# zhxie0117/video-tokenizer

Hardware: AMD Instinct MI355X
Metric: clips/sec (16x128x128) tokenizer fwd+bwd (higher is better)
Workload: dtype bf16; 1 GPU; cfgs/larp_tokenizer.yaml base geometry as LARPTokenizer(bottleneck_type=vq): config B, 16x128x128 clips, 8 clips/GPU, 12+12 blocks, Nq=1024, d=24, K=8192, stochastic VQ (tau 0.03), loss = L1 + 0.1*loss_q; global_batch=8, parallelism=dp1

## Files before the change

### include/vt_hip.h

```cpp
#ifndef VT_HIP_H
#define VT_HIP_H
#include <stddef.h>
#include <stdint.h>
#ifdef __cplusplus
extern "C" {
#endif

typedef void* vtStream;

enum { VT_OK = 0, VT_ERR_INVALID = -1, VT_ERR_LAUNCH = -2, VT_ERR_UNSUPPORTED = -3 };

int vt_abi_version(void);
int vt_last_error(char* buf, size_t n);

typedef struct {
    int32_t grp;
    int64_t stride;
    int64_t off;
} vtRowMap;

enum {
    VT_EPI_BF16 = 0,
    VT_EPI_BF16_GELU = 1,
    VT_EPI_F32 = 2,
// ... 8 lines not shown
    int32_t M, N, K;
    int32_t epi;
    void* out; int64_t ldo;
    void* out2; int64_t ldo2;
    const float* bias;
    const float* residual; int64_t ldr;
    const float* rowmod; int32_t rowmod_period;
    const void* aux; int64_t ldaux;
    vtRowMap omap;
    int32_t round_bf16;
    float* colsum_partial;
    float out_scale;
    int32_t tile;
    void* splitk_ws; int64_t splitk_ws_bytes;
    int32_t splitk;
} vtGemmNT;
size_t vt_gemm_nt_splitk_workspace_bytes(void);

int vt_gemm_nt(const vtGemmNT* p_host, vtStream stream);

#define VT_TN_MAX_GROUP 16
typedef struct {
    const void* A; int64_t lda;
    const void* B; int64_t ldb;
    int32_t M, P, Q;
    float* out; int64_t ldo;
    int32_t p_lim, q_lim;
    const int32_t* row_perm;
    int32_t tile;
} vtGemmTN;
// ... 322 lines not shown
```

### video-tokenizer_amd/csrc/vt_attention.hip

```cpp
#include "vt_common.h"
#include <stdlib.h>

#include <type_traits>

#include "vt_attn_tile.h"

namespace {

struct AttnOps {
    const bf16_t *q, *k, *v;
    int64_t q_rs, k_rs, v_rs;
    int Lq, Lk;
};
struct AttnGrads {
    bf16_t *dq, *dk, *dv;
    int64_t dq_rs, dk_rs, dv_rs;
};
struct HeadPtrs {
    int blk;
    int Lq, Lk;
    int hq, hkv;
    int group;
    int64_t qrow, krow;
    int64_t q_rs, k_rs, v_rs, ors;
// ... 277 lines not shown
            sacc[r] = ds[0];
            sacc[r + 1] = ds[1];
        }
#pragma unroll
        for (int sp = 0; sp < 2; ++sp) {
            const bf16x8 dsf = pack8(sacc, sp);
#pragma unroll
            for (int dt = 0; dt < HD / 32; ++dt)
                dq[dt] = __builtin_amdgcn_mfma_f32_32x32x16_bf16(trfrag_a<HD>(kl, ad, kt * 32, sp, dt), dsf, dq[dt], 0, 0, 0);
        }
    }
}

template <int KS>
__device__ __forceinline__ float delta_own(const bf16x8 (&of)[KS], const bf16x8 (&dof)[KS]) {
    float d = 0.f;
#pragma unroll
    for (int s = 0; s < KS; ++s)
#pragma unroll
        for (int j = 0; j < 8; ++j) d += bf2f(of[s][j]) * bf2f(dof[s][j]);
    d += __shfl_xor(d, 32);
    return d;
}

template <int HD, bool CAUSAL, bool CROSS, bool OWN_DELTA, class Heads>
__device__ __forceinline__ void attn_bwd_dq_body(Heads&& heads, const bf16_t* __restrict__ o, const bf16_t* __restrict__ dO,
                                                 const float* __restrict__ lse2, std::conditional_t<OWN_DELTA, float, const float>* __restrict__ delta,
                                                 const AttnGrads grads, float scale, float scale_log2e, int q_begin) {
    extern __shared__ __attribute__((aligned(16))) char smem[];
    const int tid = threadIdx.x, lane = tid & 63;
    const int wave = __builtin_amdgcn_readfirstlane(tid >> 6);
    const int half = lane >> 5;
    const HeadPtrs hp = heads();
    const int Lq = hp.Lq, Lk = hp.Lk;
    const int q0 = q_begin + hp.blk * 128 + wave * 32;
// ... 280 lines not shown

template <int HD>
constexpr int kDqLds = 4 * AG<HD>::TILE;
template <int HD>
constexpr int kDkvLds = 2 * (2 * AG<HD>::TILE + 512);

template <int HD, bool CROSS = false>
static void launch_bwd(const AttnOps& ops, const void* o, const void* dO, const float* lse2, int B, int H, int q_begin, const AttnGrads& grads,
                       float* delta_ws, hipStream_t s) {
    if (q_begin > 0) {
        const int64_t n = (int64_t)B * q_begin * (H * HD / 8);
        hipLaunchKernelGGL(zero_q_rows_kernel, dim3((unsigned)((n + 255) / 256)), dim3(256), 0, s, grads.dq, ops.Lq, q_begin, (int64_t)3 * H * HD, H * HD);
    }
    const int nblk_q = (ops.Lq - q_begin + 127) / 128, nblk_k = (ops.Lk + 127) / 128;
    const int n_dq = nblk_q * B * H, n_dkv = nblk_k * B * H;
    hipLaunchKernelGGL((attn_delta_kernel<HD, CROSS>), dim3(n_dq), dim3(256), 0, s, ops, (const bf16_t*)o, (const bf16_t*)dO, delta_ws, H, nblk_q,
                       q_begin);
    hipLaunchKernelGGL((attn_bwd_kernel<HD, CROSS>), dim3(n_dkv + n_dq), dim3(256), kDqLds<HD> > kDkvLds<HD> ? kDqLds<HD> : kDkvLds<HD>, s, ops,
                       (const bf16_t*)dO, lse2, delta_ws, grads, H, nblk_q, nblk_k, n_dkv, kScale<HD>, kScaleLog2e<HD>, q_begin);
}
static void launch_causal_bwd(const AttnOps& ops, const void* o, const void* dO, const float* lse2, int B, int H, const AttnGrads& grads,
                              float* delta_ws, hipStream_t s) {
    const int nblk = (ops.Lq + 127) / 128;
    hipLaunchKernelGGL(attn_causal_bwd_dq_kernel, dim3(nblk * B * H), dim3(256), kDqLds<64>, s, ops, (const bf16_t*)o, (const bf16_t*)dO, lse2,
                       delta_ws, grads, H, nblk, kScale<64>, kScaleLog2e<64>);
    hipLaunchKernelGGL(attn_causal_bwd_dkv_kernel, dim3(nblk * B * H), dim3(256), kDkvLds<64>, s, ops, (const bf16_t*)dO, lse2, delta_ws, grads, H,
                       nblk, kScale<64>, kScaleLog2e<64>);
}

static bool attn_aligned(const void* a, const void* b = nullptr, const void* c = nullptr, const void* d = nullptr) {
    return ((((uintptr_t)a) | ((uintptr_t)b) | ((uintptr_t)c) | ((uintptr_t)d)) & 15) == 0;
}
// ... 8 lines not shown

extern "C" int vt_attention_fwd_rows(const void* qkv, int32_t B, int32_t L, int32_t H, int32_t hd, int32_t q_begin, void* o_compact, float* lse2,
                                     vtStream stream) {
    VT_CHECK_ARG(qkv && o_compact && lse2, "vt_attention_fwd: null pointer");
    VT_CHECK_ARG(attn_aligned(qkv, o_compact), "vt_attention_fwd: qkv and o must be 16-byte aligned");
    int rc = attn_check("vt_attention_fwd", B, L, H, hd, q_begin);
    if (rc) return rc;
    if (hd == 64) launch_fwd<64>(packed_ops(qkv, L), B, H, q_begin, o_compact, lse2, (hipStream_t)stream);
    else launch_fwd<32>(packed_ops(qkv, L), B, H, q_begin, o_compact, lse2, (hipStream_t)stream);
    VT_CHECK_LAUNCH("vt_attention_fwd");
    return VT_OK;
}

extern "C" int vt_attention_bwd_rows(const void* qkv, const void* o_compact, const void* dO_compact, const float* lse2, int32_t B, int32_t L,
                                     int32_t H, int32_t hd, int32_t q_begin, void* dqkv, float* delta_ws, vtStream stream) {
    VT_CHECK_ARG(qkv && o_compact && dO_compact && lse2 && dqkv && delta_ws, "vt_attention_bwd: null pointer");
    VT_CHECK_ARG(attn_aligned(qkv, o_compact, dO_compact, dqkv), "vt_attention_bwd: qkv, o, dO and dqkv must be 16-byte aligned");
    int rc = attn_check("vt_attention_bwd", B, L, H, hd, q_begin);
    if (rc) return rc;
    if (hd == 64) launch_bwd<64>(packed_ops(qkv, L), o_compact, dO_compact, lse2, B, H, q_begin, packed_grads(dqkv), delta_ws, (hipStream_t)stream);
    else launch_bwd<32>(packed_ops(qkv, L), o_compact, dO_compact, lse2, B, H, q_begin, packed_grads(dqkv), delta_ws, (hipStream_t)stream);
    VT_CHECK_LAUNCH("vt_attention_bwd");
    return VT_OK;
}

extern "C" int vt_attention_fwd(const void* qkv, int32_t B, int32_t L, int32_t H, int32_t hd, void* o, float* lse2, vtStream stream) {
    return vt_attention_fwd_rows(qkv, B, L, H, hd, 0, o, lse2, stream);
}

extern "C" int vt_attention_bwd(const void* qkv, const void* o, const void* dO, const float* lse2, int32_t B, int32_t L, int32_t H,
                                int32_t hd, void* dqkv, float* delta_ws, vtStream stream) {
// ... 140 lines not shown
```

### video-tokenizer_amd/csrc/vt_common.h

```cpp
#pragma once
#include <hip/hip_runtime.h>
#include <stdint.h>
#include <stdio.h>
#include <string.h>

#include "../../include/vt_hip.h"

typedef __bf16 bf16_t;
typedef __attribute__((ext_vector_type(8))) __bf16 bf16x8;
typedef __attribute__((ext_vector_type(4))) __bf16 bf16x4;
typedef __attribute__((ext_vector_type(2))) __bf16 bf16x2;
typedef __attribute__((ext_vector_type(4))) short s16x4;
typedef __attribute__((ext_vector_type(2))) float f32x2;
typedef __attribute__((ext_vector_type(4))) float f32x4;
typedef __attribute__((ext_vector_type(16))) float f32x16;

#define VT_LDS __attribute__((address_space(3)))
#define VT_GLB __attribute__((address_space(1)))

void vt_set_error(const char* fmt, ...);
#define VT_CHECK_ARG(cond, ...)                 \
    do {                                        \
        if (!(cond)) {                          \
            vt_set_error(__VA_ARGS__);          \
// ... 144 lines not shown
    const int q = nwg >> 3, r = nwg & 7, x = bid & 7;
    const int base = (x < r) ? x * (q + 1) : r * (q + 1) + (x - r) * q;
    return base + (bid >> 3);
}

static inline int vt_auto_col_block(int tiles_n, int in_flight) {
    if (tiles_n < 2 || in_flight < 4) return 0;
    int target = 1;
    while ((target + 1) * (target + 1) <= in_flight) ++target;
    if ((target + 1) * (target + 1) - in_flight < in_flight - target * target) ++target;
    int k = (tiles_n + target / 2) / target;
    if (k < 1) k = 1;
    const int w = (tiles_n + k - 1) / k;
    return w >= tiles_n ? 0 : w;
}
__host__ __device__ __forceinline__ void vt_tile_of(int sid, int tiles_m, int tiles_n, int col_block, int& tm, int& tn) {
    tm = sid / tiles_n, tn = sid - tm * tiles_n;
    if (col_block > 0) {
        const int per = tiles_m * col_block, b = sid / per, r = sid - b * per;
        const int left = tiles_n - b * col_block, w = left < col_block ? left : col_block;
        tm = r / w, tn = b * col_block + (r - tm * w);
    }
}

struct RowMap {
    int grp;
    int64_t stride, off;
    __host__ __device__ __forceinline__ int64_t operator()(int64_t r) const {
        return grp ? (r / grp) * stride + off + (r % grp) : r;
    }
// ... 18 lines not shown
```

### video-tokenizer_amd/csrc/vt_engine.hip

```cpp
#include <vector>

#include "vt_common.h"

extern "C" int vt_kl_forward(const float* z, int64_t ldz, int64_t M, int32_t d, int32_t batch, uint64_t seed, const uint32_t* seed_counter,
                             float* mean, float* sample, void* sample_pad_bf16, int64_t ldp, float* noise, float* loss_kl, void* workspace,
                             vtStream stream) __attribute__((weak));
extern "C" int vt_kl_backward(const float* g_sample, int64_t ldg, const float* g_mean, const float* gkl, const float* z, int64_t ldz,
                              const float* noise, int64_t M, int32_t d, int32_t batch, float* dz, void* dz_pad_bf16, int64_t ldp,
                              vtStream stream) __attribute__((weak));
extern "C" int vt_rope_rotate(void* qkv, int64_t ld, int64_t M, int32_t L, int32_t H, const float* cos_tab, const float* sin_tab,
                              int32_t conjugate, vtStream stream) __attribute__((weak));

static const bool g_no_splitk = [] { const char* e = getenv("VT_GEMM_SPLITK"); return e && strcmp(e, "0") == 0; }();

namespace {

__global__ void gather_f32_kernel(const float* __restrict__ src, const int32_t* __restrict__ perm, int n, float* __restrict__ dst) {
    const int i = blockIdx.x * blockDim.x + threadIdx.x;
    if (i < n) dst[i] = src[perm[i]];
}
__global__ void scatter_f32_kernel(const float* __restrict__ src, const int32_t* __restrict__ perm, int n, float* __restrict__ dst) {
    const int i = blockIdx.x * blockDim.x + threadIdx.x;
    if (i < n) dst[perm[i]] = src[i];
}
// ... 206 lines not shown
        t->vq_ws = a.take(vt_vq_workspace_bytes(t->Mq, c.K, c.d));
    }
    t->encoded_int = a.take(Mqp * D * 4);
    t->hN = a.take(Mvp * D * 2); t->meanH = a.take(Mvp * 4); t->rstdH = a.take(Mvp * 4);
    t->yrows = a.take(Mvp * Kp * 4);
    for (Side* sd : {&t->enc, &t->dec}) {
        const int nk = sd == &t->enc ? c.Nq : t->Nv, q_begin = t->L - nk;
        sd->last.rows = Rows{{nk, t->L, q_begin}, c.B * nk, (int)round_up(c.B * nk, 128), q_begin};
        sd->last.enabled = q_begin % 64 == 0 && q_begin > 0;
    }
    plan_block_scratch(t, a, {&t->enc, &t->dec}, (int)(Kp > (size_t)t->D4 ? Kp : t->D4));
    t->dY = a.take(Mvp * Kp * 2); t->dhN = a.take(Mvp * D * 2);
    t->dEncb = a.take(Mqp * D * 2); t->d_rz = a.take(Mqp * 64 * 4); t->dz_pad = a.take(Mqp * 64 * 2);
    t->dTok = a.take(Mvp * D * 2);
    t->tmp_vec = a.take((Kp > (size_t)t->D4 ? Kp : t->D4) * 4);
    t->wg_slabs = a.take((size_t)16 * D * 64 * 4);
    t->ws_bytes = a.off;
    *out = t;
    return VT_OK;
}

extern "C" int vt_tokenizer_create(const vtTokenizerConfig* cfg, vtTokenizer** out) { return create_tokenizer(cfg, false, out); }
extern "C" int vt_tokenizer_create_kl(const vtTokenizerConfig* cfg, vtTokenizer** out) { return create_tokenizer(cfg, true, out); }

extern "C" void vt_tokenizer_destroy(vtTokenizer* t) { delete t; }
extern "C" size_t vt_tokenizer_workspace_bytes(const vtTokenizer* t) { return t ? t->ws_bytes : 0; }
extern "C" int32_t vt_tokenizer_num_backward_stages(const vtTokenizer* t) { return t ? 3 + t->c.depth_enc + t->c.depth_dec : 0; }
static int set_split_k(BlockEngine* e, int32_t on, const char* fn) {
    VT_CHECK_ARG(e, "%s: null handle", fn);
    e->splitk_on = on != 0;
    return VT_OK;
// ... 230 lines not shown
                         WS(float, t->meanH), WS(float, t->rstdH), s));
    vtGemmNT g = nt(t, ws, WS(void, t->hN), D, WS(void, t->head_wb), D, t->Mv, t->Kp, D, VT_EPI_F32, WS(void, t->yrows), t->Kp);
    g.bias = WS(float, t->head_b_perm);
    TRY(vt_gemm_nt(&g, s));
    TRY(vt_unpatchify(WS(float, t->yrows), c.B, c.C, c.T, c.S, c.pt, c.p, pred, s));
    return VT_OK;
}

static vtGemmTN tn(const void* A, int64_t lda, const void* B, int64_t ldb, int M, int P, int Q, float* out, int64_t ldo) {
    vtGemmTN p;
    memset(&p, 0, sizeof(p));
    p.A = A; p.lda = lda; p.B = B; p.ldb = ldb; p.M = M; p.P = P; p.Q = Q; p.out = out; p.ldo = ldo; p.p_lim = P; p.q_lim = Q;
    return p;
}

static int skinny_wgrad(vtTokenizer* t, vtGemmTN w, void* ws, vtStream s) {
    int ns = 16;
    while (ns > 1 && (w.M % (64 * ns)) != 0) ns >>= 1;
    if (ns == 1) return vt_gemm_tn_grouped(&w, 1, s);
    const int rows = w.M / ns;
    const size_t slab = (size_t)w.p_lim * w.q_lim;
    vtGemmTN pr[16];
    float* part = WS(float, t->wg_slabs);
    for (int i = 0; i < ns; ++i) {
        pr[i] = w;
        pr[i].A = (const char*)w.A + (size_t)i * rows * w.lda * 2;
        pr[i].B = (const char*)w.B + (size_t)i * rows * w.ldb * 2;
        pr[i].M = rows;
        pr[i].out = part + i * slab;
        pr[i].ldo = w.q_lim;
    }
    TRY(vt_gemm_tn_grouped(pr, ns, s));
// ... 77 lines not shown
    void* dqkv = WS(void, g0.dqkv);
    if (kept) TRY(vt_cast_rows(dX, r.map, r.n, D, dXa, D, s));
    vtGemmNT g = nt(e, ws, dXa, D, WS(void, b.fc2_wt), D, r.n, D4, D, VT_EPI_BF16_MULAUX, du, D4);
    g.aux = WS(void, b.dgelu); g.ldaux = D4;
    g.colsum_partial = WS(float, g0.cs_part);
    TRY(vt_gemm_nt(&g, s));
    queue_slab_sum(e, WS(float, g0.cs_part), (r.n + 191) / 192, D4, gr.fc1_b);
    g = nt(e, ws, du, D4, WS(void, b.fc1_wt), D4, r.n, D, D4, VT_EPI_BF16, WS(void, e->dh), D);
    TRY(vt_gemm_nt(&g, s));
    int nsl = 0;
    TRY(vt_layernorm_bwd_partials(WS(void, e->dh), WS(float, b.x_mid), r.map, w.norm2_w, WS(float, b.mean2), WS(float, b.rstd2), dX, r.n, D, dX,
                                  kept ? nullptr : dXm, WS(float, g0.ln_part2), &nsl, s));
    queue_ln_reduce(e, WS(float, g0.ln_part2), nsl, D, gr.norm2_w, gr.norm2_b, gr.proj_b);
    if (kept) TRY(vt_cast_rows(dX, r.map, r.n, D, dXm, D, s));
    g = nt(e, ws, dXm, D, WS(void, b.proj_wt), D, r.n, D, D, VT_EPI_BF16, WS(void, e->dob), D);
    TRY(vt_gemm_nt(&g, s));
    TRY(attn_bwd(e, ws, WS(void, b.qkv), WS(void, b.o), WS(void, e->dob), WS(float, b.lse), r.q_begin, dqkv, s));
    if (rope_cos) TRY(vt_rope_rotate(dqkv, D3, M, e->L, e->H, rope_cos, rope_sin, 1, s));
    g = nt(e, ws, dqkv, D3, WS(void, b.qkv_wt), D3, M, D, D3, VT_EPI_BF16, WS(void, e->dh), D);
    TRY(vt_gemm_nt(&g, s));
    e->pending.push_back(tn(dXa, D, WS(void, b.g), D4, r.n_pad, D, D4, gr.fc2_w, D4));
    e->pending.push_back(tn(du, D4, WS(void, b.h2), D, r.n_pad, D4, D, gr.fc1_w, D));
    e->pending.push_back(tn(dXm, D, WS(void, b.o), D, r.n_pad, D, D, gr.proj_w, D));
    e->pending.push_back(tn(dqkv, D3, WS(void, b.h1), D, Mp, D3, D, gr.qkv_w, D));
    e->pending_blocks++;
    TRY(vt_layernorm_bwd_partials(WS(void, e->dh), x_in, id, w.norm1_w, WS(float, b.mean1), WS(float, b.rstd1), dX, M, D, dX, WS(void, g1.dx_out),
                                  WS(float, g0.ln_part1), &nsl, s));
    queue_ln_reduce(e, WS(float, g0.ln_part1), nsl, D, gr.norm1_w, gr.norm1_b, prev_bias_grad);
    e->set_idx = set_next;
    return VT_OK;
}

// ... 34 lines not shown
            t->pending_red.clear(); t->pending_blocks = 0; t->set_idx = 0; t->final_through = 0;
            t->sets_pending.clear();
            TRY(join_wgrad_stream(t, s));
            VT_CHECK_ARG(d_pred, "vt_tokenizer_backward: stage 0 needs d_pred");
            TRY(vt_patchify(d_pred, c.B, c.C, c.T, c.S, c.pt, c.p, WS(void, t->dY), s));
            vtGemmNT g = nt(t, ws, WS(void, t->dY), Kp, WS(void, t->head_wt), Kp, t->Mv, D, Kp, VT_EPI_BF16, WS(void, t->dhN), D);
            TRY(vt_gemm_nt(&g, s));
            vtGemmTN w = tn(WS(void, t->dY), Kp, WS(void, t->hN), D, t->Mvp, Kp, D, G->head_w, D);
            w.row_perm = WS(int32_t, t->perm);
            TRY(vt_gemm_tn_grouped(&w, 1, s));
            TRY(vt_colsum(WS(void, t->dY), 1, Kp, id, t->Mv, Kp, WS(float, t->tmp_vec), WS(void, t->cs_ws), s));
            hipLaunchKernelGGL(scatter_f32_kernel, dim3((Kp + 255) / 256), dim3(256), 0, hs, WS(float, t->tmp_vec), WS(int32_t, t->perm), Kp, G->head_b);
            TRY(vt_zero_rows(dX, WS(void, t->gs[0].dx_out), lmap, t->Mq, D, s));
            TRY(vt_layernorm_bwd(WS(void, t->dhN), WS(float, t->dec.x[c.depth_dec]), vmap, P->head_norm_w, WS(float, t->meanH), WS(float, t->rstdH),
                                 nullptr, t->Mv, D, dX, WS(void, t->gs[0].dx_out), G->head_norm_w, G->head_norm_b,
                                 nullptr, WS(void, t->ln_ws), s));
            TRY(vt_colsum(dX, 0, D, id, t->M, D, G->dec_blocks[c.depth_dec - 1].fc2_b, WS(void, t->cs_ws), s));
            t->final_through = 1;
        } else if (st <= c.depth_dec) {
            const int i = c.depth_dec - st;
            TRY(backward_block_stage(t, t->dec, i, P->dec_blocks, G->dec_blocks, true, false, st + 1, ws, s));
        } else if (st == c.depth_dec + 1) {
            if (G->dec_token_type) TRY(vt_colsum(dX, 0, D, vmap, t->Mv, D, G->dec_token_type, WS(void, t->cs_ws), s));
            TRY(vt_cast_rows(dX, lmap, t->Mq, D, WS(void, t->dEncb), D, s));
            TRY(vt_colsum(WS(void, t->dEncb), 1, D, id, t->Mq, D, G->out_b, WS(void, t->cs_ws), s));
            vtGemmNT g = nt(t, ws, WS(void, t->dEncb), D, WS(void, t->out_wt), D, t->Mq, 64, D, VT_EPI_F32, WS(void, t->d_rz), 64);
            TRY(vt_gemm_nt(&g, s));
            vtGemmTN w = tn(WS(void, t->dEncb), D, WS(void, t->vq_rzpad), 64, t->Mqp, D, 64, G->out_w, c.d);
            w.q_lim = c.d;
            TRY(skinny_wgrad(t, w, ws, s));
            const int pd = t->kl ? 2 * c.d : c.d;
            if (t->kl) {
// ... 12 lines not shown
            TRY(wait_set(t, t->set_idx, s));
            TRY(vt_zero_rows(dX, WS(void, t->gs[t->set_idx].dx_out), tmap, t->Mv, D, s));
            g = nt(t, ws, WS(void, t->dz_pad), 64, WS(void, t->in_wt), 64, t->Mq, D, 64, VT_EPI_F32, dX, D);
            g.out2 = WS(void, t->gs[t->set_idx].dx_out); g.ldo2 = D; g.omap = qmap;
            TRY(vt_gemm_nt(&g, s));
            TRY(vt_colsum(dX, 0, D, id, t->M, D, G->enc_blocks[c.depth_enc - 1].fc2_b, WS(void, t->cs_ws), s));
            t->final_through = st + 1;
        } else if (st <= c.depth_dec + 1 + c.depth_enc) {
            const int i = c.depth_enc - (st - c.depth_dec - 1);
            TRY(backward_block_stage(t, t->enc, i, P->enc_blocks, G->enc_blocks, true, i < t->wg_tail, st + 1, ws, s));
        } else {
            TRY(vt_batch_sum(dX, qmap, c.B, Nq, D, G->enc_query, s));
            TRY(vt_cast_rows(dX, tmap, t->Mv, D, WS(void, t->dTok), D, s));
            TRY(vt_colsum(WS(void, t->dTok), 1, D, id, t->Mv, D, G->pe_b, WS(void, t->cs_ws), s));
            vtGemmTN w = tn(WS(void, t->dTok), D, WS(void, t->patches), Kp, t->Mvp, D, Kp, G->pe_w, Kp);
            TRY(vt_gemm_tn_grouped(&w, 1, s));
            TRY(join_wgrad_stream(t, s));
            t->final_through = st + 1;
        }
    }
    if (final_through) *final_through = t->final_through;
    VT_CHECK_LAUNCH("vt_tokenizer_backward");
    return VT_OK;
}

extern "C" int vt_tokenizer_backward_until_flush(vtTokenizer* t, const vtTokenizerTensors* P, const float* d_pred, const float* gscal, void* ws,
                                                 const vtTokenizerTensors* G, int32_t stage_begin, int32_t* stage_next, int32_t* final_through,
                                                 vtStream s) {
    VT_CHECK_ARG(t && stage_next && final_through, "vt_tokenizer_backward_until_flush: null pointer");
    const int nstage = vt_tokenizer_num_backward_stages(t);
    VT_CHECK_ARG(stage_begin >= 0 && stage_begin < nstage, "vt_tokenizer_backward_until_flush: bad first stage");
// ... 96 lines not shown
```

### video-tokenizer_amd/csrc/vt_gemm.hip

```cpp
#include "vt_common.h"
#include "vt_gemm_epilogue.h"

namespace {

constexpr int BM = 128, BN = 128, BK = 64;
constexpr int TILE_B = BM * BK * 2;

struct NTArgs {
    vtGemmNT p;
    int tiles_m, tiles_n;
    int col_block;
    int split;
    float* part;
    unsigned* ctr;
};

__device__ __forceinline__ void st_part(float* p, const f32x4& v) {
    asm volatile("global_store_dwordx4 %0, %1, off sc1\n\ts_nop 1" ::"v"(p), "v"(v) : "memory");
}

__device__ __forceinline__ void stage_nt(const bf16_t* __restrict__ g, int64_t ld, int row0, int nrows, int k0,
                                         char* lds, int tid, int wave) {
#pragma unroll
    for (int i = 0; i < 4; ++i) {
// ... 465 lines not shown
    VT_CHECK_ARG(p.M > 0 && p.N > 0 && p.K > 0 && p.K % BK == 0, "vt_gemm_nt: K=%d must be a positive multiple of 64 (M=%d N=%d)", p.K, p.M, p.N);
    VT_CHECK_ARG(p.lda % 8 == 0 && p.ldb % 8 == 0 && p.lda >= p.K && p.ldb >= p.K, "vt_gemm_nt: lda/ldb must be >= K and multiples of 8");
    VT_CHECK_ARG(((uintptr_t)p.A & 15) == 0 && ((uintptr_t)p.B & 15) == 0, "vt_gemm_nt: A/B must be 16-byte aligned");
    VT_CHECK_ARG(p.ldo % 4 == 0, "vt_gemm_nt: ldo must be a multiple of 4");
    VT_CHECK_ARG(((uintptr_t)p.out & 15) == 0 && ((uintptr_t)p.bias & 15) == 0 && ((uintptr_t)p.out2 & 7) == 0 &&
                 ((uintptr_t)p.residual & 15) == 0 && ((uintptr_t)p.rowmod & 15) == 0 && ((uintptr_t)p.aux & 7) == 0,
                 "vt_gemm_nt: out/bias/residual/rowmod must be 16-byte aligned (out2/aux 8-byte)");
    VT_CHECK_ARG(!p.rowmod || p.N % 4 == 0, "vt_gemm_nt: rowmod needs N %% 4 == 0");
    if (p.epi == VT_EPI_BF16_GELU) VT_CHECK_ARG(p.out2 && p.ldo2 % 4 == 0, "vt_gemm_nt: GELU epilogue needs out2");
    if (p.epi == VT_EPI_BF16_GELU_GRAD) VT_CHECK_ARG(p.out2 && p.ldo2 % 4 == 0, "vt_gemm_nt: GELU_GRAD epilogue needs out2");
    if (p.epi == VT_EPI_BF16_DGELU) VT_CHECK_ARG(p.aux && p.ldaux % 4 == 0, "vt_gemm_nt: DGELU epilogue needs aux");
    if (p.epi == VT_EPI_BF16_MULAUX) VT_CHECK_ARG(p.aux && p.ldaux % 4 == 0, "vt_gemm_nt: MULAUX epilogue needs aux");
    VT_CHECK_ARG(p.out_scale == 0.f || p.epi == VT_EPI_F32, "vt_gemm_nt: out_scale only with VT_EPI_F32");
    VT_CHECK_ARG(!p.colsum_partial || ((p.epi == VT_EPI_BF16_DGELU || p.epi == VT_EPI_BF16_MULAUX) && p.N % 4 == 0),
                 "vt_gemm_nt: colsum_partial needs the DGELU or MULAUX epilogue and N %% 4 == 0 (it always runs on the 192-row tile kernel)");
    if (p.epi == VT_EPI_F32) {
        VT_CHECK_ARG(!p.residual || p.ldr % 4 == 0, "vt_gemm_nt: ldr must be a multiple of 4");
        VT_CHECK_ARG(!p.rowmod || p.rowmod_period > 0, "vt_gemm_nt: rowmod needs a period");
        VT_CHECK_ARG(!p.out2 || p.ldo2 % 4 == 0, "vt_gemm_nt: ldo2 must be a multiple of 4");
    } else {
        VT_CHECK_ARG(p.omap.grp == 0, "vt_gemm_nt: output row map only with VT_EPI_F32");
    }
    if (tile.kernel == NTTile::SKINNY || (tile.kernel == NTTile::AUTO && p.M <= 64 && !p.colsum_partial && p.N >= 64)) {
        VT_CHECK_ARG(p.M <= 64 && !p.colsum_partial, "vt_gemm_nt: tile 7 (skinny) needs M <= 64 and no colsum_partial (M=%d)", p.M);
        hipStream_t s = (hipStream_t)stream;
        TRY(dispatch_epi(p.epi, [&](auto epi) { launch_skinny<decltype(epi)::value>(p, s); return VT_OK; }));
        VT_CHECK_LAUNCH("vt_gemm_nt(skinny)");
        return VT_OK;
    }
    bool big = tile.kernel == NTTile::T192 || p.colsum_partial;
    if (tile.kernel == NTTile::AUTO && !big && p.N >= 192 && p.M >= 192) {
        const long t192 = (long)((p.M + 191) / 192) * ((p.N + 191) / 192), t128 = (long)((p.M + BM - 1) / BM) * ((p.N + BN - 1) / BN);
        const double c192 = (double)((t192 + 255) / 256);
        const long rem = t128 % 512;
        const double last = rem == 0 ? 0.0 : rem <= 256 ? 0.6 : 0.6 + 0.4 * (double)(rem - 256) / 256.0;
        const double c128 = 1.05 * ((double)(t128 / 512) + last);
        big = c192 <= c128;
    }
    if (big) {
        TRY(vt_gemm192_init());
        TRY(vt_gemm_nt192_launch(p, (hipStream_t)stream, tile.one_tile, tile.order));
        VT_CHECK_LAUNCH("vt_gemm_nt(192)");
        return VT_OK;
    }
    NTArgs a;
    a.p = p;
    a.tiles_m = (p.M + BM - 1) / BM;
    a.tiles_n = (p.N + BN - 1) / BN;
    a.split = 1; a.part = nullptr; a.ctr = nullptr;
    const int tiles = a.tiles_m * a.tiles_n;
    hipStream_t s = (hipStream_t)stream;
    const int n_cu = vt_gemm_num_cus();
    const int nt_all = p.K / BK;
// ... 78 lines not shown
```

### video-tokenizer_amd/csrc/vt_gemm192.hip

```cpp
#include <stdlib.h>

#include "vt_common.h"
#include "vt_gemm_epilogue.h"

namespace {

constexpr int TM = 192, TN_ = 192, TK = 64;
constexpr int OP_BYTES = TM * TK * 2;
constexpr int STAGE_BYTES = 2 * OP_BYTES;
constexpr int NSTAGE = 3;
constexpr int THREADS = 512;
constexpr int PA = 3, PB = 3, P = PA + PB;

__device__ __forceinline__ void wait_vmcnt6() { asm volatile("s_waitcnt vmcnt(6)" ::: "memory"); }
static_assert(P == 6 && PA * THREADS == TM * 8 && PB * THREADS == TN_ * 8, "wait_vmcnt6 counts one K-tile");
__device__ __forceinline__ void wait_vmcnt0() { asm volatile("s_waitcnt vmcnt(0)" ::: "memory"); }
__device__ __forceinline__ void raw_barrier() {
    asm volatile("" ::: "memory");
    __builtin_amdgcn_s_barrier();
    asm volatile("" ::: "memory");
}

struct NT192Args {
    vtGemmNT p;
// ... 67 lines not shown
        for (int g = 0; g < 3; ++g) {
            const int m = m0 + row, n = n0 + col0 + g * 64;
            if (m >= p.M || n >= p.N) continue;
            V* const o = (V*)((bf16_t*)p.out + (int64_t)m * p.ldo + n);
            auto o2 = [&] { return (V*)((bf16_t*)p.out2 + (int64_t)m * p.ldo2 + n); };
            if constexpr (EPI == VT_EPI_BF16_GELU_GRAD) {
                V gl, dg;
                gelu_grad_lookup<VEC>(hh[g], tab, gl, dg);
                st_stream_any(o, dg);
                st_stream_any(o2(), gl);
            } else {
                st_stream_any(o, hh[g]);
                if constexpr (EPI == VT_EPI_BF16_GELU) st_stream_any(o2(), gelu_lookup<VEC>(hh[g], (const bf16_t*)tab));
            }
        }
    }
}

__device__ __forceinline__ void nt192_piece_offsets(int64_t lda, int m0, int M, int64_t ldb, int n0, int N, int tid, unsigned (&off)[P]) {
#pragma unroll
    for (int piece = 0; piece < P; ++piece) {
        const bool isA = piece < PA;
        const int i = isA ? piece : piece - PA;
        const int slot = i * THREADS + tid;
        const int row = slot >> 3;
        const int lc = (slot & 7) ^ ((row >> 1) & 7);
        const int r0 = isA ? m0 : n0, lim = isA ? M : N;
        int gr = r0 + row;
        gr = (gr < lim ? gr : lim - 1) - r0;
        off[piece] = (unsigned)((gr * (isA ? lda : ldb) + lc * 8) * 2);
// ... 235 lines not shown
                    }
                }
                if (p.colsum_partial) {
                    float* red = (float*)(smem + TM * IMG_STRIDE);
                    if (rl < RL) *(f32x4*)(red + rl * TN_ + c * 4) = cs;
                    __syncthreads();
                    if (tid_e < TN_ && en0 + tid_e < p.N) {
                        float sum = 0.f;
#pragma unroll
                        for (int r = 0; r < RL; ++r) sum += red[r * TN_ + tid_e];
                        p.colsum_partial[(int64_t)(em0 / TM) * p.N + en0 + tid_e] = sum;
                    }
                }
                continue;
            }
            if ((p.N & 7) == 0 && (p.ldo & 7) == 0 && ((EPI != VT_EPI_BF16_GELU && !GG) || (p.ldo2 & 7) == 0)) nt192_read_back<EPI, 8>(p, smem, tab, tid_e, em0, en0);
            else nt192_read_back<EPI, 4>(p, smem, tab, tid_e, em0, en0);
            continue;
        }
    }
    const RowMap omap{p.omap.grp, p.omap.stride, p.omap.off};
    int tid_x = tid;
    asm volatile("" : "+v"(tid_x));
    const int fr_x = tid_x & 15, fq_x = (tid_x & 63) >> 4;
    if constexpr (EPI == VT_EPI_F32) {
        if ((p.N & 3) == 0) {
            constexpr int FSTRIDE = TN_ * 4 + 16;
            f32x4 b4[3];
#pragma unroll
            for (int j = 0; j < 3; ++j) {
                const int n = en0 + wn * 48 + j * 16 + fq_x * 4;
                b4[j] = (p.bias && n < p.N) ? *(const f32x4*)(p.bias + n) : (f32x4){0.f, 0.f, 0.f, 0.f};
// ... 458 lines not shown
```

### video-tokenizer_amd/hip.py

```python
import ctypes
import os

import torch

_HERE = os.path.dirname(os.path.abspath(__file__))
LIB_PATH = os.environ.get("VT_HIP_LIB") or os.path.join(_HERE, "libvt_hip.so")
_lib = None

c_i32, c_i64, c_f32, c_u64, c_vp, c_sz = ctypes.c_int32, ctypes.c_int64, ctypes.c_float, ctypes.c_uint64, ctypes.c_void_p, ctypes.c_size_t

EPI_BF16, EPI_BF16_GELU, EPI_F32, EPI_BF16_DGELU, EPI_BF16_GELU_GRAD, EPI_BF16_MULAUX = 0, 1, 2, 3, 4, 5
TN_MAX_GROUP = 16


class RowMap(ctypes.Structure):
    _fields_ = [("grp", c_i32), ("stride", c_i64), ("off", c_i64)]


IDENT = RowMap(0, 0, 0)


class GemmNT(ctypes.Structure):
    _fields_ = [("A", c_vp), ("lda", c_i64), ("B", c_vp), ("ldb", c_i64), ("M", c_i32), ("N", c_i32), ("K", c_i32),
                ("epi", c_i32), ("out", c_vp), ("ldo", c_i64), ("out2", c_vp), ("ldo2", c_i64), ("bias", c_vp),
                ("residual", c_vp), ("ldr", c_i64), ("rowmod", c_vp), ("rowmod_period", c_i32), ("aux", c_vp),
                ("ldaux", c_i64), ("omap", RowMap), ("round_bf16", c_i32), ("colsum_partial", c_vp), ("out_scale", c_f32), ("tile", c_i32),
                ("splitk_ws", c_vp), ("splitk_ws_bytes", c_i64), ("splitk", c_i32)]


class GemmTN(ctypes.Structure):
    _fields_ = [("A", c_vp), ("lda", c_i64), ("B", c_vp), ("ldb", c_i64), ("M", c_i32), ("P", c_i32), ("Q", c_i32),
                ("out", c_vp), ("ldo", c_i64), ("p_lim", c_i32), ("q_lim", c_i32), ("row_perm", c_vp), ("tile", c_i32)]

class Clip(ctypes.Structure):
    _fields_ = [("data", c_vp), ("T", c_i32), ("H", c_i32), ("W", c_i32)]


GEMM_TILE = 0


SIGNATURES = {
    "vt_abi_version": (c_i32, []),
# ... 250 lines not shown

GEMM_SPLITK = True
_SPLITK_WS = {}


def splitk_workspace(dev):
    key = (dev.index if dev.index is not None else torch.cuda.current_device(), torch.cuda.current_stream(dev).cuda_stream)
    ws = _SPLITK_WS.get(key)
    if ws is None:
        ws = torch.zeros(lib().vt_gemm_nt_splitk_workspace_bytes(), device=dev, dtype=torch.uint8)
        _SPLITK_WS[key] = ws
    return ws


def gemm_nt(A, B, epi=EPI_BF16, bias=None, out=None, out2=None, residual=None, rowmod=None, rowmod_period=0,
            aux=None, omap=None, round_bf16=False, out_rows=None, colsum_partial=None, tile=None, out_scale=0.0, splitk=1):
    require_gpu(A, B)
    assert A.dtype == torch.bfloat16 and B.dtype == torch.bfloat16
    M, K = A.shape
    N = B.shape[0]
    dev = A.device
    if out is None:
        rows = out_rows if out_rows is not None else M
        out = torch.empty(rows, N, device=dev, dtype=torch.float32 if epi == EPI_F32 else torch.bfloat16)
    if epi in (EPI_BF16_GELU, EPI_BF16_GELU_GRAD) and out2 is None:
        out2 = torch.empty(M, N, device=dev, dtype=torch.bfloat16)
    p = GemmNT()
    p.A, p.lda, p.B, p.ldb = A.data_ptr(), A.stride(0), B.data_ptr(), B.stride(0)
    p.M, p.N, p.K, p.epi = M, N, K, epi
    p.out, p.ldo = out.data_ptr(), out.stride(0)
    p.out2, p.ldo2 = (out2.data_ptr(), out2.stride(0)) if out2 is not None else (None, 0)
    p.bias = bias.data_ptr() if bias is not None else None
    p.residual, p.ldr = (residual.data_ptr(), residual.stride(0)) if residual is not None else (None, 0)
    p.rowmod, p.rowmod_period = (rowmod.data_ptr(), rowmod_period) if rowmod is not None else (None, 0)
    p.aux, p.ldaux = (aux.data_ptr(), aux.stride(0)) if aux is not None else (None, 0)
    p.omap = omap if omap is not None else IDENT
    p.round_bf16 = int(round_bf16)
    p.colsum_partial = colsum_partial.data_ptr() if colsum_partial is not None else None
    p.tile = GEMM_TILE if tile is None else tile
    p.out_scale = float(out_scale)
    if splitk != 1 and GEMM_SPLITK:
        ws = splitk_workspace(dev)
        p.splitk_ws, p.splitk_ws_bytes, p.splitk = ws.data_ptr(), ws.numel(), 0 if splitk is None else int(splitk)
    else:
        p.splitk_ws, p.splitk_ws_bytes, p.splitk = None, 0, 1
    check(lib().vt_gemm_nt(ctypes.byref(p), stream()), "vt_gemm_nt")
    return (out, out2) if epi in (EPI_BF16_GELU, EPI_BF16_GELU_GRAD) else out


def gemm_tn_grouped(problems):
    arr = (GemmTN * len(problems))()
    for i, pr in enumerate(problems):
        A, B, out = pr["A"], pr["B"], pr["out"]
        g = arr[i]
        g.A, g.lda, g.B, g.ldb = A.data_ptr(), A.stride(0), B.data_ptr(), B.stride(0)
# ... 900 lines not shown
```

Measured before the change: 361.0 clips/s.

## Fuse attention-backward delta rowdot into dO projection GEMM epilogue

The projection-backward GEMM that produces dO now also computes the per-row, per-head dot product of dO with the saved attention output O in its 192-tile epilogue and writes it to the delta buffer, so the separate attention delta kernel is skipped when that tile is chosen. The change also folds the final fc2 bias column-sum into the layernorm backward call and splits the patch-embed weight gradient into slabs via skinny_wgrad with a larger slab workspace. This removes one kernel launch and a re-read of O and dO per block in exchange for extra register pressure and global loads in the GEMM epilogue, and it forces the 192 tile whenever rowdot is requested.

```diff
diff --git a/include/vt_hip.h b/include/vt_hip.h
--- a/include/vt_hip.h
+++ b/include/vt_hip.h
@@ -46,6 +46,9 @@
     int32_t tile;
     void* splitk_ws; int64_t splitk_ws_bytes;
     int32_t splitk;
+    const void* rowdot_with; int64_t ld_rowdot;
+    float* rowdot_out;
+    int32_t rowdot_hd, rowdot_H, rowdot_L, rowdot_q_begin;
 } vtGemmNT;
 size_t vt_gemm_nt_splitk_workspace_bytes(void);
 
diff --git a/video-tokenizer_amd/csrc/vt_attention.hip b/video-tokenizer_amd/csrc/vt_attention.hip
--- a/video-tokenizer_amd/csrc/vt_attention.hip
+++ b/video-tokenizer_amd/csrc/vt_attention.hip
@@ -4,6 +4,7 @@
 #include <type_traits>
 
 #include "vt_attn_tile.h"
+#include "vt_rowdot.h"
 
 namespace {
 
@@ -315,11 +316,7 @@
 
 template <int KS>
 __device__ __forceinline__ float delta_own(const bf16x8 (&of)[KS], const bf16x8 (&dof)[KS]) {
-    float d = 0.f;
-#pragma unroll
-    for (int s = 0; s < KS; ++s)
-#pragma unroll
-        for (int j = 0; j < 8; ++j) d += bf2f(of[s][j]) * bf2f(dof[s][j]);
+    float d = rowdot_chain<KS>(of, dof);
     d += __shfl_xor(d, 32);
     return d;
 }
@@ -630,8 +627,9 @@
     }
     const int nblk_q = (ops.Lq - q_begin + 127) / 128, nblk_k = (ops.Lk + 127) / 128;
     const int n_dq = nblk_q * B * H, n_dkv = nblk_k * B * H;
-    hipLaunchKernelGGL((attn_delta_kernel<HD, CROSS>), dim3(n_dq), dim3(256), 0, s, ops, (const bf16_t*)o, (const bf16_t*)dO, delta_ws, H, nblk_q,
-                       q_begin);
+    if (o)
+        hipLaunchKernelGGL((attn_delta_kernel<HD, CROSS>), dim3(n_dq), dim3(256), 0, s, ops, (const bf16_t*)o, (const bf16_t*)dO, delta_ws, H, nblk_q,
+                           q_begin);
     hipLaunchKernelGGL((attn_bwd_kernel<HD, CROSS>), dim3(n_dkv + n_dq), dim3(256), kDqLds<HD> > kDkvLds<HD> ? kDqLds<HD> : kDkvLds<HD>, s, ops,
                        (const bf16_t*)dO, lse2, delta_ws, grads, H, nblk_q, nblk_k, n_dkv, kScale<HD>, kScaleLog2e<HD>, q_begin);
 }
@@ -670,7 +668,7 @@
 
 extern "C" int vt_attention_bwd_rows(const void* qkv, const void* o_compact, const void* dO_compact, const float* lse2, int32_t B, int32_t L,
                                      int32_t H, int32_t hd, int32_t q_begin, void* dqkv, float* delta_ws, vtStream stream) {
-    VT_CHECK_ARG(qkv && o_compact && dO_compact && lse2 && dqkv && delta_ws, "vt_attention_bwd: null pointer");
+    VT_CHECK_ARG(qkv && dO_compact && lse2 && dqkv && delta_ws, "vt_attention_bwd: null pointer");
     VT_CHECK_ARG(attn_aligned(qkv, o_compact, dO_compact, dqkv), "vt_attention_bwd: qkv, o, dO and dqkv must be 16-byte aligned");
     int rc = attn_check("vt_attention_bwd", B, L, H, hd, q_begin);
     if (rc) return rc;
diff --git a/video-tokenizer_amd/csrc/vt_common.h b/video-tokenizer_amd/csrc/vt_common.h
--- a/video-tokenizer_amd/csrc/vt_common.h
+++ b/video-tokenizer_amd/csrc/vt_common.h
@@ -182,6 +182,15 @@
     const int w = (tiles_n + k - 1) / k;
     return w >= tiles_n ? 0 : w;
 }
+static inline bool vt_nt_auto_192(int M, int N) {
+    if (N < 192 || M < 192) return false;
+    const long t192 = (long)((M + 191) / 192) * ((N + 191) / 192), t128 = (long)((M + 127) / 128) * ((N + 127) / 128);
+    const double c192 = (double)((t192 + 255) / 256);
+    const long rem = t128 % 512;
+    const double last = rem == 0 ? 0.0 : rem <= 256 ? 0.6 : 0.6 + 0.4 * (double)(rem - 256) / 256.0;
+    const double c128 = 1.05 * ((double)(t128 / 512) + last);
+    return c192 <= c128;
+}
 __host__ __device__ __forceinline__ void vt_tile_of(int sid, int tiles_m, int tiles_n, int col_block, int& tm, int& tn) {
     tm = sid / tiles_n, tn = sid - tm * tiles_n;
     if (col_block > 0) {
diff --git a/video-tokenizer_amd/csrc/vt_engine.hip b/video-tokenizer_amd/csrc/vt_engine.hip
--- a/video-tokenizer_amd/csrc/vt_engine.hip
+++ b/video-tokenizer_amd/csrc/vt_engine.hip
@@ -244,7 +244,7 @@
     t->dEncb = a.take(Mqp * D * 2); t->d_rz = a.take(Mqp * 64 * 4); t->dz_pad = a.take(Mqp * 64 * 2);
     t->dTok = a.take(Mvp * D * 2);
     t->tmp_vec = a.take((Kp > (size_t)t->D4 ? Kp : t->D4) * 4);
-    t->wg_slabs = a.take((size_t)16 * D * 64 * 4);
+    t->wg_slabs = a.take(((size_t)16 * D * 64 > (size_t)8 * D * Kp ? (size_t)16 * D * 64 : (size_t)8 * D * Kp) * 4);
     t->ws_bytes = a.off;
     *out = t;
     return VT_OK;
@@ -505,8 +505,8 @@
     return p;
 }
 
-static int skinny_wgrad(vtTokenizer* t, vtGemmTN w, void* ws, vtStream s) {
-    int ns = 16;
+static int skinny_wgrad(vtTokenizer* t, vtGemmTN w, void* ws, vtStream s, int max_slabs = 16) {
+    int ns = max_slabs;
     while (ns > 1 && (w.M % (64 * ns)) != 0) ns >>= 1;
     if (ns == 1) return vt_gemm_tn_grouped(&w, 1, s);
     const int rows = w.M / ns;
@@ -614,8 +614,13 @@
     queue_ln_reduce(e, WS(float, g0.ln_part2), nsl, D, gr.norm2_w, gr.norm2_b, gr.proj_b);
     if (kept) TRY(vt_cast_rows(dX, r.map, r.n, D, dXm, D, s));
     g = nt(e, ws, dXm, D, WS(void, b.proj_wt), D, r.n, D, D, VT_EPI_BF16, WS(void, e->dob), D);
-    TRY(vt_gemm_nt(&g, s));
-    TRY(attn_bwd(e, ws, WS(void, b.qkv), WS(void, b.o), WS(void, e->dob), WS(float, b.lse), r.q_begin, dqkv, s));
+    const bool delta_from_gemm = g.tile == 6 || (g.tile == 0 && r.n > 64 && vt_nt_auto_192(r.n, D));
+    if (delta_from_gemm) {
+        g.rowdot_with = WS(void, b.o); g.ld_rowdot = D; g.rowdot_out = WS(float, e->delta);
+        g.rowdot_hd = D / e->H; g.rowdot_H = e->H; g.rowdot_L = e->L; g.rowdot_q_begin = r.q_begin;
+    }
+    TRY(vt_gemm_nt(&g, s));
+    TRY(attn_bwd(e, ws, WS(void, b.qkv), delta_from_gemm ? nullptr : WS(void, b.o), WS(void, e->dob), WS(float, b.lse), r.q_begin, dqkv, s));
     if (rope_cos) TRY(vt_rope_rotate(dqkv, D3, M, e->L, e->H, rope_cos, rope_sin, 1, s));
     g = nt(e, ws, dqkv, D3, WS(void, b.qkv_wt), D3, M, D, D3, VT_EPI_BF16, WS(void, e->dh), D);
     TRY(vt_gemm_nt(&g, s));
@@ -680,8 +685,7 @@
             TRY(vt_zero_rows(dX, WS(void, t->gs[0].dx_out), lmap, t->Mq, D, s));
             TRY(vt_layernorm_bwd(WS(void, t->dhN), WS(float, t->dec.x[c.depth_dec]), vmap, P->head_norm_w, WS(float, t->meanH), WS(float, t->rstdH),
                                  nullptr, t->Mv, D, dX, WS(void, t->gs[0].dx_out), G->head_norm_w, G->head_norm_b,
-                                 nullptr, WS(void, t->ln_ws), s));
-            TRY(vt_colsum(dX, 0, D, id, t->M, D, G->dec_blocks[c.depth_dec - 1].fc2_b, WS(void, t->cs_ws), s));
+                                 G->dec_blocks[c.depth_dec - 1].fc2_b, WS(void, t->ln_ws), s));
             t->final_through = 1;
         } else if (st <= c.depth_dec) {
             const int i = c.depth_dec - st;
@@ -724,7 +728,7 @@
             TRY(vt_cast_rows(dX, tmap, t->Mv, D, WS(void, t->dTok), D, s));
             TRY(vt_colsum(WS(void, t->dTok), 1, D, id, t->Mv, D, G->pe_b, WS(void, t->cs_ws), s));
             vtGemmTN w = tn(WS(void, t->dTok), D, WS(void, t->patches), Kp, t->Mvp, D, Kp, G->pe_w, Kp);
-            TRY(vt_gemm_tn_grouped(&w, 1, s));
+            TRY(skinny_wgrad(t, w, ws, s, 8));
             TRY(join_wgrad_stream(t, s));
             t->final_through = st + 1;
         }
diff --git a/video-tokenizer_amd/csrc/vt_gemm.hip b/video-tokenizer_amd/csrc/vt_gemm.hip
--- a/video-tokenizer_amd/csrc/vt_gemm.hip
+++ b/video-tokenizer_amd/csrc/vt_gemm.hip
@@ -503,6 +503,16 @@
     VT_CHECK_ARG(p.out_scale == 0.f || p.epi == VT_EPI_F32, "vt_gemm_nt: out_scale only with VT_EPI_F32");
     VT_CHECK_ARG(!p.colsum_partial || ((p.epi == VT_EPI_BF16_DGELU || p.epi == VT_EPI_BF16_MULAUX) && p.N % 4 == 0),
                  "vt_gemm_nt: colsum_partial needs the DGELU or MULAUX epilogue and N %% 4 == 0 (it always runs on the 192-row tile kernel)");
+    const bool rowdot = p.rowdot_out || p.rowdot_with;
+    if (rowdot) {
+        VT_CHECK_ARG(p.epi == VT_EPI_BF16 && p.rowdot_out && p.rowdot_with, "vt_gemm_nt: rowdot needs the VT_EPI_BF16 epilogue, rowdot_with and rowdot_out");
+        VT_CHECK_ARG((p.rowdot_hd == 32 || p.rowdot_hd == 64) && p.rowdot_H > 0 && (int64_t)p.rowdot_H * p.rowdot_hd == p.N,
+                     "vt_gemm_nt: rowdot_hd=%d must be 32 or 64 and N=%d == rowdot_H * rowdot_hd (rowdot_H=%d)", p.rowdot_hd, p.N, p.rowdot_H);
+        VT_CHECK_ARG(p.rowdot_q_begin >= 0 && p.rowdot_q_begin < p.rowdot_L && p.M % (p.rowdot_L - p.rowdot_q_begin) == 0,
+                     "vt_gemm_nt: rowdot rows: M=%d must be a multiple of rowdot_L - rowdot_q_begin (L=%d q_begin=%d)", p.M, p.rowdot_L, p.rowdot_q_begin);
+        VT_CHECK_ARG(((uintptr_t)p.rowdot_with & 15) == 0 && p.ld_rowdot % 8 == 0 && p.ld_rowdot >= p.N && ((uintptr_t)p.rowdot_out & 3) == 0,
+                     "vt_gemm_nt: rowdot_with must be 16-byte aligned with ld_rowdot >= N a multiple of 8");
+    }
     if (p.epi == VT_EPI_F32) {
         VT_CHECK_ARG(!p.residual || p.ldr % 4 == 0, "vt_gemm_nt: ldr must be a multiple of 4");
         VT_CHECK_ARG(!p.rowmod || p.rowmod_period > 0, "vt_gemm_nt: rowmod needs a period");
@@ -510,22 +520,15 @@
     } else {
         VT_CHECK_ARG(p.omap.grp == 0, "vt_gemm_nt: output row map only with VT_EPI_F32");
     }
-    if (tile.kernel == NTTile::SKINNY || (tile.kernel == NTTile::AUTO && p.M <= 64 && !p.colsum_partial && p.N >= 64)) {
-        VT_CHECK_ARG(p.M <= 64 && !p.colsum_partial, "vt_gemm_nt: tile 7 (skinny) needs M <= 64 and no colsum_partial (M=%d)", p.M);
+    if (tile.kernel == NTTile::SKINNY || (tile.kernel == NTTile::AUTO && p.M <= 64 && !p.colsum_partial && !rowdot && p.N >= 64)) {
+        VT_CHECK_ARG(p.M <= 64 && !p.colsum_partial && !rowdot, "vt_gemm_nt: tile 7 (skinny) needs M <= 64 and no colsum_partial / rowdot (M=%d)", p.M);
         hipStream_t s = (hipStream_t)stream;
         TRY(dispatch_epi(p.epi, [&](auto epi) { launch_skinny<decltype(epi)::value>(p, s); return VT_OK; }));
         VT_CHECK_LAUNCH("vt_gemm_nt(skinny)");
         return VT_OK;
     }
-    bool big = tile.kernel == NTTile::T192 || p.colsum_partial;
-    if (tile.kernel == NTTile::AUTO && !big && p.N >= 192 && p.M >= 192) {
-        const long t192 = (long)((p.M + 191) / 192) * ((p.N + 191) / 192), t128 = (long)((p.M + BM - 1) / BM) * ((p.N + BN - 1) / BN);
-        const double c192 = (double)((t192 + 255) / 256);
-        const long rem = t128 % 512;
-        const double last = rem == 0 ? 0.0 : rem <= 256 ? 0.6 : 0.6 + 0.4 * (double)(rem - 256) / 256.0;
-        const double c128 = 1.05 * ((double)(t128 / 512) + last);
-        big = c192 <= c128;
-    }
+    bool big = tile.kernel == NTTile::T192 || p.colsum_partial || rowdot;
+    if (tile.kernel == NTTile::AUTO && !big) big = vt_nt_auto_192(p.M, p.N);
     if (big) {
         TRY(vt_gemm192_init());
         TRY(vt_gemm_nt192_launch(p, (hipStream_t)stream, tile.one_tile, tile.order));
diff --git a/video-tokenizer_amd/csrc/vt_gemm192.hip b/video-tokenizer_amd/csrc/vt_gemm192.hip
--- a/video-tokenizer_amd/csrc/vt_gemm192.hip
+++ b/video-tokenizer_amd/csrc/vt_gemm192.hip
@@ -2,6 +2,7 @@
 
 #include "vt_common.h"
 #include "vt_gemm_epilogue.h"
+#include "vt_rowdot.h"
 
 namespace {
 
@@ -105,6 +106,54 @@
                 if constexpr (EPI == VT_EPI_BF16_GELU) st_stream_any(o2(), gelu_lookup<VEC>(hh[g], (const bf16_t*)tab));
             }
         }
+    }
+}
+
+constexpr int RD_REGS = 16;
+template <int HD>
+struct RowDotGeom {
+    static constexpr int NPAIR = TM * (TN_ / HD), NIT = (NPAIR + THREADS - 1) / THREADS, CH = HD / 8, KS = HD / 16;
+    static_assert(NIT * CH <= RD_REGS && TN_ % HD == 0, "rowdot registers");
+    int row, m, n;
+    bool ok;
+    __device__ __forceinline__ RowDotGeom(const vtGemmNT& p, int it, int tid, int m0, int n0) {
+        const int pair = it * THREADS + tid, head = pair / TM;
+        row = pair - head * TM, m = m0 + row, n = n0 + head * HD;
+        ok = pair < NPAIR && m < p.M && n < p.N;
+    }
+};
+template <int HD>
+__device__ __forceinline__ void rowdot_load(const vtGemmNT& p, int tid, int m0, int n0, bf16x8 (&w)[RD_REGS]) {
+    using G = RowDotGeom<HD>;
+#pragma unroll
+    for (int it = 0; it < G::NIT; ++it) {
+        const G g(p, it, tid, m0, n0);
+        const int m = g.m < p.M ? g.m : p.M - 1, n = g.n <= p.N - HD ? g.n : p.N - HD;
+        const bf16x8* src = (const bf16x8*)((const bf16_t*)p.rowdot_with + (int64_t)m * p.ld_rowdot + n);
+#pragma unroll
+        for (int c = 0; c < G::CH; ++c) w[it * G::CH + c] = src[c];
+    }
+}
+template <int HD>
+__device__ __forceinline__ void rowdot_finish(const vtGemmNT& p, const char* img, int tid, int m0, int n0, const bf16x8 (&w)[RD_REGS]) {
+    using G = RowDotGeom<HD>;
+#pragma unroll
+    for (int it = 0; it < G::NIT; ++it) {
+        const G g(p, it, tid, m0, n0);
+        if (!g.ok) continue;
+        const char* src = img + g.row * IMG_STRIDE + (g.n - n0) * 2;
+        float d0 = 0.f, d1 = 0.f;
+#pragma unroll
+        for (int s = 0; s < G::KS; ++s) {
+            const bf16x8 o0 = cat4(*(const bf16x4*)(src + 32 * s), *(const bf16x4*)(src + 32 * s + 8));
+            const bf16x8 o1 = cat4(*(const bf16x4*)(src + 32 * s + 16), *(const bf16x4*)(src + 32 * s + 24));
+            d0 = rowdot_step(d0, w[it * G::CH + 2 * s], o0);
+            d1 = rowdot_step(d1, w[it * G::CH + 2 * s + 1], o1);
+            __builtin_amdgcn_sched_barrier(0);
+        }
+        const float d = d0 + d1;
+        const int Lo = p.rowdot_L - p.rowdot_q_begin, b = g.m / Lo, i = g.m - b * Lo;
+        p.rowdot_out[((int64_t)b * p.rowdot_H + g.n / HD) * p.rowdot_L + p.rowdot_q_begin + i] = d;
     }
 }
 
@@ -370,8 +419,27 @@
                 }
                 continue;
             }
-            if ((p.N & 7) == 0 && (p.ldo & 7) == 0 && ((EPI != VT_EPI_BF16_GELU && !GG) || (p.ldo2 & 7) == 0)) nt192_read_back<EPI, 8>(p, smem, tab, tid_e, em0, en0);
-            else nt192_read_back<EPI, 4>(p, smem, tab, tid_e, em0, en0);
+            auto read_back = [&] {
+                if ((p.N & 7) == 0 && (p.ldo & 7) == 0 && ((EPI != VT_EPI_BF16_GELU && !GG) || (p.ldo2 & 7) == 0)) nt192_read_back<EPI, 8>(p, smem, tab, tid_e, em0, en0);
+                else nt192_read_back<EPI, 4>(p, smem, tab, tid_e, em0, en0);
+            };
+            if constexpr (EPI == VT_EPI_BF16) {
+                if (p.rowdot_out && p.rowdot_hd == 64) {
+                    bf16x8 rdw[RD_REGS];
+                    rowdot_load<64>(p, tid_e, em0, en0, rdw);
+                    read_back();
+                    rowdot_finish<64>(p, smem, tid_e, em0, en0, rdw);
+                    continue;
+                }
+                if (p.rowdot_out) {
+                    bf16x8 rdw[RD_REGS];
+                    rowdot_load<32>(p, tid_e, em0, en0, rdw);
+                    read_back();
+                    rowdot_finish<32>(p, smem, tid_e, em0, en0, rdw);
+                    continue;
+                }
+            }
+            read_back();
             continue;
         }
     }
diff --git a/video-tokenizer_amd/csrc/vt_rowdot.h b/video-tokenizer_amd/csrc/vt_rowdot.h
--- /dev/null
+++ b/video-tokenizer_amd/csrc/vt_rowdot.h
@@ -0,0 +1,15 @@
+#pragma once
+#include "vt_common.h"
+
+__device__ __forceinline__ float rowdot_step(float d, const bf16x8& of, const bf16x8& dof) {
+#pragma unroll
+    for (int j = 0; j < 8; ++j) d += bf2f(of[j]) * bf2f(dof[j]);
+    return d;
+}
+template <int KS>
+__device__ __forceinline__ float rowdot_chain(const bf16x8 (&of)[KS], const bf16x8 (&dof)[KS]) {
+    float d = 0.f;
+#pragma unroll
+    for (int s = 0; s < KS; ++s) d = rowdot_step(d, of[s], dof[s]);
+    return d;
+}
diff --git a/video-tokenizer_amd/hip.py b/video-tokenizer_amd/hip.py
--- a/video-tokenizer_amd/hip.py
+++ b/video-tokenizer_amd/hip.py
@@ -25,7 +25,9 @@
                 ("epi", c_i32), ("out", c_vp), ("ldo", c_i64), ("out2", c_vp), ("ldo2", c_i64), ("bias", c_vp),
                 ("residual", c_vp), ("ldr", c_i64), ("rowmod", c_vp), ("rowmod_period", c_i32), ("aux", c_vp),
                 ("ldaux", c_i64), ("omap", RowMap), ("round_bf16", c_i32), ("colsum_partial", c_vp), ("out_scale", c_f32), ("tile", c_i32),
-                ("splitk_ws", c_vp), ("splitk_ws_bytes", c_i64), ("splitk", c_i32)]
+                ("splitk_ws", c_vp), ("splitk_ws_bytes", c_i64), ("splitk", c_i32),
+                ("rowdot_with", c_vp), ("ld_rowdot", c_i64), ("rowdot_out", c_vp), ("rowdot_hd", c_i32), ("rowdot_H", c_i32),
+                ("rowdot_L", c_i32), ("rowdot_q_begin", c_i32)]
 
 
 class GemmTN(ctypes.Structure):
@@ -306,7 +308,7 @@
 
 
 def gemm_nt(A, B, epi=EPI_BF16, bias=None, out=None, out2=None, residual=None, rowmod=None, rowmod_period=0,
-            aux=None, omap=None, round_bf16=False, out_rows=None, colsum_partial=None, tile=None, out_scale=0.0, splitk=1):
+            aux=None, omap=None, round_bf16=False, out_rows=None, colsum_partial=None, tile=None, out_scale=0.0, splitk=1, rowdot=None):
     require_gpu(A, B)
     assert A.dtype == torch.bfloat16 and B.dtype == torch.bfloat16
     M, K = A.shape
@@ -331,6 +333,9 @@
     p.colsum_partial = colsum_partial.data_ptr() if colsum_partial is not None else None
     p.tile = GEMM_TILE if tile is None else tile
     p.out_scale = float(out_scale)
+    if rowdot is not None:
+        p.rowdot_with, p.ld_rowdot, p.rowdot_out = rowdot["with_"].data_ptr(), rowdot["with_"].stride(0), rowdot["out"].data_ptr()
+        p.rowdot_hd, p.rowdot_H, p.rowdot_L, p.rowdot_q_begin = rowdot["hd"], rowdot["H"], rowdot["L"], rowdot.get("q_begin", 0)
     if splitk != 1 and GEMM_SPLITK:
         ws = splitk_workspace(dev)
         p.splitk_ws, p.splitk_ws_bytes, p.splitk = ws.data_ptr(), ws.numel(), 0 if splitk is None else int(splitk)
```

Measured after the change: 362.3 clips/s, median of 6. Within noise of the previous version (+0.4%).
